# jeertmans/DiffeRT2d

Measured on AMD Instinct MI355X. Metric: ray-path candidates/s, higher is better.
Workload: dtype f32

## Files before the change

differt2d_amd/csrc/d2d.hip:

```cpp
#include <hip/hip_runtime.h>
#include <dlfcn.h>
#include <rccl/rccl.h>

#include <algorithm>
#include <cmath>
#include <cstdarg>
#include <cstdio>
#include <cstring>
#include <string>
#include <cstdlib>
#include <vector>

#include "../../include/d2d.h"
#define D2D_AUX_KERNELS 1
#include "d2d_launch.hpp"
#include "d2d_host.hpp"
#include "d2d_own.hpp"
#include "d2d_optgrad.hpp"
#include "d2d_optrev.hpp"

namespace d2d {

#define D2D_BY_MODE(fn, ...)                                   \
    switch (mode) {                                            \
// ... 273 lines not shown
        float tx = dx - ox, ty = dy - oy;
        float vx = ty, vy = -tx;
        float len = sqrtf(vx * vx + vy * vy);
        if (len == 0.0f) len = 1.0f;
        float nx = vx / len, ny = vy / len;
        float sq = tx * tx + ty * ty;
        if (sq == 0.0f) sq = 1.0f;
        refl[2 * j] = make_float4(ox, oy, nx, ny);
        refl[2 * j + 1] = make_float4(tx, ty, sq, len);
        const double rsq = 1.0 / (double)sq;
        flt[j] = make_float4((float)rsq, (float)(64.0 * 1.1920929e-07 * rsq), 0.0f, 0.0f);
    }
    int rc = c->d_refl.ensure(refl.size());
    if (rc) return rc;
    if ((rc = c->d_flt.ensure(flt.size()))) return rc;
    HIP_TRY(hipMemcpyAsync(c->d_flt.p, flt.data(), flt.size() * sizeof(float4), hipMemcpyHostToDevice, c->stream));
    if ((rc = c->d_kind.ensure((size_t)c->N + 1))) return rc;
    if ((rc = c->d_sincos.ensure((size_t)c->N + 1))) return rc;
    if ((rc = c->d_xys.ensure((size_t)c->N + 1))) return rc;
    if (c->N > 0) HIP_TRY(hipMemcpyAsync(c->d_xys.p, c->xys.data(), (size_t)c->N * sizeof(float4), hipMemcpyHostToDevice, c->stream));
    std::vector<float2> sc((size_t)c->N + 1);
    for (int j = 0; j < c->N; ++j) sc[(size_t)j] = make_float2(sinf(c->phi[j]), cosf(c->phi[j]));
    HIP_TRY(hipMemcpyAsync(c->d_refl.p, refl.data(), refl.size() * sizeof(float4), hipMemcpyHostToDevice, c->stream));
    if (c->N > 0) {
        HIP_TRY(hipMemcpyAsync(c->d_kind.p, c->kind.data(), (size_t)c->N, hipMemcpyHostToDevice, c->stream));
        HIP_TRY(hipMemcpyAsync(c->d_sincos.p, sc.data(), (size_t)c->N * sizeof(float2), hipMemcpyHostToDevice, c->stream));
    }
    HIP_TRY(hipStreamSynchronize(c->stream));
    return D2D_OK;
}

int upload_occl(d2d_ctx* c, float patch) {
    if (c->occl_patch == patch && c->d_occl.p) return D2D_OK;
    std::vector<float4> occl((size_t)c->N + 1);
    for (int j = 0; j < c->N; ++j) {
        const float* w = &c->xys[4 * (size_t)j];
        float ox = w[0], oy = w[1], dx = w[2], dy = w[3];
        float tx = dx - ox, ty = dy - oy;
        float ptx = patch * tx, pty = patch * ty;
        float p1x = ox - ptx, p1y = oy - pty;
        float p2x = dx + ptx, p2y = dy + pty;
        occl[j] = make_float4(p1x, p1y, p2x - p1x, p2y - p1y);
    }
    int rc = c->d_occl.ensure(occl.size());
    if (rc) return rc;
    HIP_TRY(hipMemcpyAsync(c->d_occl.p, occl.data(), occl.size() * sizeof(float4), hipMemcpyHostToDevice, c->stream));
    HIP_TRY(hipStreamSynchronize(c->stream));
    c->occl_patch = patch;
    return D2D_OK;
}

int upload_mask(d2d_ctx* c) {
    c->cw.clear();
    for (int j = 0; j < c->N; ++j)
        if (c->allowed[j]) c->cw.push_back(j);
    int rc = c->d_cw.ensure(c->cw.size() + 1);
    if (rc) return rc;
    if (!c->cw.empty()) {
        HIP_TRY(hipMemcpyAsync(c->d_cw.p, c->cw.data(), c->cw.size() * sizeof(int), hipMemcpyHostToDevice, c->stream));
        HIP_TRY(hipStreamSynchronize(c->stream));
    }
    return D2D_OK;
}

d2d::ObjTables obj_tables(d2d_ctx* c) {
    d2d::ObjTables T;
    T.occl = c->d_occl.p;
// ... 801 lines not shown
        if (c->stream) HIP_TRY(hipStreamSynchronize(c->stream));
        if (c->aux_stream) HIP_TRY(hipStreamSynchronize(c->aux_stream));
        if (c->sort_stream) HIP_TRY(hipStreamSynchronize(c->sort_stream));
        c->for_each_set([](d2d_ctx::PrepSet& sp) { sp.swept_pending = false; });
        c->last_small = small;
    }
    s.piped = c->pipeline && c->aux_stream != nullptr && s.d_stats == nullptr && !small;
    if (s.piped) {
        std::swap(c->cur, c->spare_sets[0]);
        for (int i = 0; i + 1 < d2d_ctx::N_SPARE; ++i) std::swap(c->spare_sets[i], c->spare_sets[i + 1]);
        s.set_was_swept = c->cur.swept_pending;
        if (c->cur.swept_pending) HIP_TRY(hipStreamWaitEvent(c->aux_stream, c->cur.ev_swept, 0));
        c->cur.swept_pending = false;
    }
    s.ps = s.piped ? c->aux_stream : c->stream;
    return D2D_OK;
}

static int sweep_args(d2d_ctx* c, Sweep& s) {
    const d2d_params* p = s.p;
    d2d::SweepArgs& a = s.a;
    memset(&a, 0, sizeof a);
    a.occl = c->d_occl.p;
    a.refl = c->d_refl.p;
    a.flt = c->d_flt.p;
    a.cw = c->d_cw.p;
    a.N = c->N;
    a.Nc = (int)c->cw.size();
    a.X = c->d_X.p;
    a.Y = c->d_Y.p;
    a.out = c->d_out.p;
    a.m = c->m;
    a.n = c->n;
    a.txx = s.tx[0];
    a.txy = s.tx[1];
    a.min_order = p->min_order;
    a.max_order = p->max_order;
    a.alpha = p->alpha;
    a.tol = p->tol;
    a.seg_lo = -p->seg_tol;
    a.seg_hi = 1.0f + p->seg_tol;
    const bool per_object = p->fun_id == D2D_FUN_RECEIVED_POWER_PER_OBJECT;
    s.th = d2d_host::sweep_thresholds(*p, s.grad_mode != 0, per_object ? c->coef.data() : nullptr, c->allowed.data(), c->N);
    a.coef = per_object ? c->d_coef.p : nullptr;
    a.flt_lo = s.th.flt_lo;
    a.flt_hi = s.th.flt_hi;
    a.on_lo = s.th.on_lo;
    a.on_hi = s.th.on_hi;
    a.loss_skip = s.th.loss_skip;
    for (int k = 0; k <= D2D_MAX_ORDER; ++k) a.fnum[k] = s.th.fnum[k];
    a.h2 = s.th.h2;
    a.sig_l2f = s.th.sig_l2f;
    a.sig_mono = s.th.sig_mono;
    a.fun_id = p->fun_id;
    a.cust_f = c->d_cust_f.p;
    a.cust_pb = c->d_cust_pb.p;
    a.cust_cells = (long)c->m * c->n;
    a.out_mode = p->out_mode;
    a.patch = p->patch;
    a.stats = s.d_stats;
    a.wave_cycles = (s.d_stats && c->want_wave_cycles) ? s.d_stats + D2D_NUM_STATS : nullptr;
    if (s.tiles > 0x7fffffffLL) return fail(D2D_ERR_INVALID, "grid too large: %lld tiles", s.tiles);
    s.grid_patches = dim3((unsigned)s.tiles);
    s.txg = p->grid_role == D2D_GRID_TX;
    const bool txg_cullable = s.txg && !c->txg_exhaustive && !(s.grad_mode && p->strict_nan);
    s.txg_culled = txg_cullable && s.th.degenerate_invalid;
// ... 127 lines not shown
    const size_t lds_l = (size_t)(3 * c->N + 1) * sizeof(float4) + 512;
    const size_t lds_r = (size_t)(3 * c->N + 1) * sizeof(float4) + (size_t)d2d::RL_GATHER * sizeof(unsigned long long);
    if (!rp.on || lds_l > d2d_host::LDS_LIMIT || lds_r > d2d_host::LDS_LIMIT) return D2D_OK;
    if (cur.d_rl_pool.ensure((size_t)rp.max_chunks * d2d::RL_CHUNK) != D2D_OK || cur.d_rl_next.ensure((size_t)rp.max_chunks) != D2D_OK) {
        (void)hipGetLastError();
        cur.d_rl_pool.release();
        cur.d_rl_next.release();
        c->rl_pool_mb = std::max<long long>(1, c->rl_pool_mb / 4);
        return D2D_OK;
    }
    const int orders = p->max_order - rp.k_lo + 1;
    const size_t per_order = (size_t)rp.leaf.slots + (size_t)rp.top.slots;
    if ((rc = cur.d_rl_idx.ensure(per_order * (size_t)orders))) return rc;
    int* const meta = reinterpret_cast<int*>(cur.d_shadow.p + c->N + d2d::SCHED_KEYS);
    cur.rl_meta_ptr = meta;
    if ((rc = cur.d_rl_meta.ensure((size_t)s.tiles))) return rc;
    if ((rc = cur.d_rl.ensure(1))) return rc;
    {
        const long long key[4] = {c->grid_version, rp.leaf.R, rp.top.R, (long long)c->m * 0x100000000ll + c->n};
        const size_t nbox = (size_t)rp.leaf.regions + (size_t)rp.top.regions;
        if (std::memcmp(key, c->rl_box_key, sizeof key) != 0 || c->d_rl_box.n < nbox) {
            if ((rc = c->d_rl_box.ensure(nbox))) return rc;
            hipLaunchKernelGGL(d2d::region_box_kernel, dim3((unsigned)rp.leaf.regions), dim3(256), 0, s.ps, c->d_X.p, c->d_Y.p,
                               c->m, c->n, rp.leaf.R, rp.leaf.regions_x, c->d_rl_box.p);
            hipLaunchKernelGGL(d2d::region_box_kernel, dim3((unsigned)rp.top.regions), dim3(256), 0, s.ps, c->d_X.p, c->d_Y.p,
                               c->m, c->n, rp.top.R, rp.top.regions_x, c->d_rl_box.p + rp.leaf.regions);
            HIP_TRY(hipGetLastError());
            std::memcpy(c->rl_box_key, key, sizeof key);
        }
    }
    auto fill = [](d2d::RegionLevel& l, const d2d_host::RegionLevelPlan& lp_) {
        l.S = lp_.S;
        l.R = lp_.R;
        l.regions_x = lp_.regions_x;
        l.regions_y = lp_.regions_y;
    };
    d2d::RegionLists rl;
    d2d::RegionLevel top;
    memset(&rl, 0, sizeof rl);
    memset(&top, 0, sizeof top);
    fill(rl.leaf, rp.leaf);
    fill(top, rp.top);
    rl.leaf.box = c->d_rl_box.p;
    top.box = c->d_rl_box.p + rp.leaf.regions;
    if ((rc = prep_hidden_masks(c, s, pr, rp, rl.leaf))) return rc;
    int* at = cur.d_rl_idx.p;
    int chunk_at = 0;
    for (int k = rp.k_lo; k <= p->max_order; ++k) {
        rl.leaf.cnt[k] = at; at += rp.leaf.slots;
        rl.leaf.chunk0[k] = chunk_at; chunk_at += (int)rp.leaf.slots;
        top.cnt[k] = at; at += rp.top.slots;
        top.chunk0[k] = chunk_at; chunk_at += (int)rp.top.slots;
    }
    rl.lp.pool = cur.d_rl_pool.p;
    rl.lp.next = cur.d_rl_next.p;
    rl.lp.head = meta + 1;
    rl.lp.n_static = (int)rp.n_static;
    rl.lp.max_chunks = (int)rp.max_chunks;
    rl.flag = meta + 2;
    a.fb_n = meta;
    a.fb_list = cur.d_rl_meta.p;
    if (!cur.rl_host_valid || std::memcmp(&rl, &cur.rl_host, sizeof rl) != 0) {
        cur.rl_host = rl;
        cur.rl_host_valid = true;
        hipLaunchKernelGGL(d2d::write_region_lists_kernel, dim3(1), dim3(1), 0, s.ps, cur.d_rl.p, rl);
        HIP_TRY(hipGetLastError());
// ... 1312 lines not shown
```

differt2d_amd/csrc/d2d_kernels.hpp:

```cpp
#pragma once
#include <hip/hip_runtime.h>
#include <stdint.h>

#include "../../include/d2d.h"

namespace d2d {

template <typename T>
__device__ __forceinline__ const __attribute__((address_space(4))) T* cmem(const T* p) {
    return (const __attribute__((address_space(4))) T*)(unsigned long long)p;
}

__device__ __forceinline__ float4 ldc4(const float4* p, long i) {
    typedef float v4f __attribute__((ext_vector_type(4)));
    const v4f v = ((const __attribute__((address_space(4))) v4f*)(unsigned long long)p)[i];
    return make_float4(v.x, v.y, v.z, v.w);
}
__device__ __forceinline__ int4 ldc4i(const int4* p, long i) {
    typedef int v4i __attribute__((ext_vector_type(4)));
    const v4i v = ((const __attribute__((address_space(4))) v4i*)(unsigned long long)p)[i];
    return make_int4(v.x, v.y, v.z, v.w);
}

template <typename T, unsigned OFF>
__device__ __forceinline__ T late_kernarg() {
    static_assert(sizeof(T) == 4 || sizeof(T) == 8, "one or two dwords");
    const auto base = __builtin_amdgcn_kernarg_segment_ptr();
    T v;
    if constexpr (sizeof(T) == 8) asm volatile("s_load_dwordx2 %0, %1, %2\n\ts_waitcnt lgkmcnt(0)" : "=s"(v) : "s"(base), "i"(OFF));
    else asm volatile("s_load_dword %0, %1, %2\n\ts_waitcnt lgkmcnt(0)" : "=s"(v) : "s"(base), "i"(OFF));
    return v;
}
#define D2D_LATE_ARG(T, field) late_kernarg<T, (unsigned)__builtin_offsetof(SweepArgs, field)>()

enum Mode { MODE_HARD = 0, MODE_HSIG = 1, MODE_SIG = 2 };

constexpr int RL_CHUNK = 128;
struct ListPool {
    unsigned long long* pool;
    int* next;
    int* head;
    int n_static;
    int max_chunks;
};
struct RegionLevel {
    int* cnt[D2D_MAX_ORDER + 1];
    int chunk0[D2D_MAX_ORDER + 1];
    int S;
    int R;
    int regions_x, regions_y;
    const float4* box;
    const unsigned long long* hidden;
    float hidden_dperp;
};
struct RegionLists {
    RegionLevel leaf;
    ListPool lp;
    int* flag;
};

struct SweepArgs {
    const RegionLists* __restrict__ rl;
    int* fb_n;
    int* fb_list;
    const float4* __restrict__ occl;
    const float4* __restrict__ refl;
    const float4* __restrict__ flt;
    const int* __restrict__ cw;
    int N, Nc;
    const float* __restrict__ X;
    const float* __restrict__ Y;
    float* __restrict__ out;
    int m, n;
    float txx, txy;
    int min_order, max_order;
    float alpha, tol;
    float seg_lo, seg_hi;
    float flt_lo, flt_hi;
    float on_lo, on_hi;
    float loss_skip;
    float sig_l2f;
    int sig_mono;
    const unsigned long long* __restrict__ shadow;
    float shadow_dperp;
    float shadow_lo, shadow_inv;
    int shadow_prefix_ok;
    const unsigned long long* __restrict__ pair;
    float pair_dperp;
    int pair_prefix_ok;
    float fnum[D2D_MAX_ORDER + 1];
    float h2;
    int fun_id;
    int out_mode;
    float patch;
    float* __restrict__ grad;
    const float* __restrict__ cot;
    float* __restrict__ partial;
    const float* __restrict__ cust_f;
    const float* __restrict__ cust_pb;
    long cust_cells;
    const float* __restrict__ coef;
    float* __restrict__ coef_partial;
    int coef_lds_off;

    const int* __restrict__ sched;
    int cullq_off;
// ... 403 lines not shown
        }
        if (K >= 2 && a.pair != nullptr) {
#pragma unroll
            for (int i = 0; i + 1 < K; ++i) {
                const unsigned long long m = HOIST ? pm_pre[i] : cmem(a.pair)[(size_t)cand[i] * a.N + cand[i + 1]];
                if (m != 0ull) {
                    const float k8 = 0.125f * a.shadow_inv;
                    const float ea_ = (sv[i] - padv[i] - a.shadow_lo) * k8, eb_ = (sv[i] + padv[i] - a.shadow_lo) * k8;
                    const float la_ = (sv[i + 1] - padv[i + 1] - a.shadow_lo) * k8, lb_ = (sv[i + 1] + padv[i + 1] - a.shadow_lo) * k8;
                    const bool ok = ea_ >= 0.0f && eb_ < 8.0f && la_ >= 0.0f && lb_ < 8.0f && 512.0f * eps * Ei[i] <= a.pair_dperp &&
                                    512.0f * eps * Ei[i + 1] <= a.pair_dperp;
                    const int ea = ok ? (int)ea_ : 0, eb = ok ? (int)eb_ : 0, la = ok ? (int)la_ : 0, lb = ok ? (int)lb_ : 0;
                    const bool all4 = ((m >> (ea + 8 * la)) & 1ull) && ((m >> (eb + 8 * la)) & 1ull) && ((m >> (ea + 8 * lb)) & 1ull) &&
                                      ((m >> (eb + 8 * lb)) & 1ull);
                    occl = occl || (ok && all4 && (eb - ea <= 1) && (lb - la <= 1));
                }
            }
        }
        if (wave_any(occl)) {
            if (MODE == MODE_HARD) hit_b = hit_b || occl;
            else if (MODE == MODE_HSIG) hit_c = occl ? 6.0f : hit_c;
            else {
                hit_z = occl ? 1.0e30f : hit_z;
                any_test = true;
            }
            active = active && (!occl || bad);
            D2D_WORK(2);
            if (!wave_any(active)) return;
        }
    }
    if (STATS) stat_add<2>(st, 1);
    constexpr bool PAIRS = MODE != MODE_SIG;
    if constexpr (PAIRS) {
    auto filt = [&](const float4& ww, int jj) -> unsigned {
        unsigned wbits = 0u;
#pragma unroll
        for (int i = 0; i <= K; ++i) {
            const int ig0 = (i == 0) ? -1 : cand[i - 1];
            const int ig1 = (i == K) ? -1 : cand[i];
            const bool skip = (jj == ig0 || jj == ig1);
            float Cx = ww.x - px[i], Cy = ww.y - py[i];
            float fa = by[i] * Cx - bx[i] * Cy;
            float fb = ww.z * Cy - ww.w * Cx;
            float fd = ww.w * bx[i] - ww.z * by[i];
            float pa = __builtin_fmaf(-a.flt_lo, fd, fa) * __builtin_fmaf(-a.flt_hi, fd, fa);
            float pb = __builtin_fmaf(-a.flt_lo, fd, fb) * __builtin_fmaf(-a.flt_hi, fd, fb);
            bool miss = fmaxf(pa, pb) > 0.0f;
            if (MODE == MODE_SIG && !skip) any_test = true;
            if (STATS) stat_add<4>(st, skip ? 0 : 1);
            wbits |= (!skip && active && (!miss || bad)) ? (1u << i) : 0u;
        }
        return wbits;
    };
    auto exact = [&](const float4& ww, int jj, unsigned wbits) {
#pragma unroll
        for (int i = 0; i <= K; ++i) {
            if (!wave_any((wbits >> i) & 1u)) continue;
            if (STATS) stat_add<5>(st, 1);
            D2D_WORK(2);
            const float Cx = ww.x - px[i], Cy = ww.y - py[i];
            const float fa = by[i] * Cx - bx[i] * Cy;
            const float fb = ww.z * Cy - ww.w * Cx;
            const float fd = ww.w * bx[i] - ww.z * by[i];
            bool dz = (fd == 0.0f);
            float dd = dz ? 1.0f : fd;
            float ta, tb;
            div2_exact(fa, fb, dd, ta, tb);
            ta = dz ? __builtin_inff() : ta;
            tb = dz ? __builtin_inff() : tb;
            if (MODE == MODE_HARD) {
                bool h = (ta >= a.seg_lo) && (ta <= a.seg_hi) && (tb >= a.seg_lo) && (tb <= a.seg_hi);
                hit_b = hit_b || h;
            } else if (MODE == MODE_HSIG) {
                nanflag = nanflag || (ta != ta) || (tb != tb);
                float c = fminf(fminf(clampact(ta - a.seg_lo, a.alpha), clampact(a.seg_hi - ta, a.alpha)),
                                fminf(clampact(tb - a.seg_lo, a.alpha), clampact(a.seg_hi - tb, a.alpha)));
                if (GRAD && (c > hit_c || (c == hit_c && hit_j >= 0 && (jj < hit_j || (jj == hit_j && i < hit_i))))) {
                    hit_i = i;
                    hit_j = jj;
                }
                if (GRAD) hit2 = (c > hit_c) ? hit_c : fmaxf(hit2, c);
                hit_c = fmaxf(hit_c, c);
            } else {
                nanflag = nanflag || (ta != ta) || (tb != tb);
                float z = fminf(fminf(a.alpha * (ta - a.seg_lo), a.alpha * (a.seg_hi - ta)),
                                fminf(a.alpha * (tb - a.seg_lo), a.alpha * (a.seg_hi - tb)));
                if (GRAD && (z > hit_z || (z == hit_z && hit_j >= 0 && (jj < hit_j || (jj == hit_j && i < hit_i))))) {
                    hit_i = i;
                    hit_j = jj;
                }
                if (GRAD) hit2 = (z > hit_z) ? hit_z : fmaxf(hit2, z);
                hit_z = fmaxf(hit_z, z);
            }
        }
        if (MODE == MODE_HARD) active = active && (!hit_b || bad);
        else if (MODE == MODE_HSIG) active = active && (hit_c != 6.0f || bad);
        else active = active && (hit_z < 17.5f || bad);
    };
    {
        bool done = a.N <= 0;
        if (!done && sh >= 0) {
            const unsigned b0 = filt(w, sh);
            D2D_WORK(K + 1);
            if (wave_any(b0 != 0u)) {
                exact(w, sh, b0);
                if (!wave_any(active)) {
                    st.shadow = sh;
                    done = true;
                }
            }
        }
        auto next_idx = [&](int x) -> int {
            ++x;
            return x == sh ? x + 1 : x;
        };
        int jA = (sh == 0) ? 1 : 0;
        if (!done && jA < a.N) {
            int jB = next_idx(jA);
            float4 wA = (sh >= 0) ? ldc4(a.occl, jA) : w;
            float4 wB = ldc4(a.occl, jB < a.N ? jB : jA);
            while (true) {
                const bool hasB = jB < a.N;
                const int nA = next_idx(jB), nB = next_idx(nA);
                const float4 wnA = ldc4(a.occl, nA < a.N ? nA : jA), wnB = ldc4(a.occl, nB < a.N ? nB : jA);
                const unsigned ba = filt(wA, jA);
                const unsigned bb = hasB ? filt(wB, jB) : 0u;
                D2D_WORK(hasB ? 2 * (K + 1) : (K + 1));
                if (wave_any((ba | bb) != 0u)) {
                    if (wave_any(ba != 0u)) {
                        exact(wA, jA, ba);
                        if (!wave_any(active)) {
                            st.shadow = jA;
                            break;
                        }
                    }
                    if (wave_any(bb != 0u)) {
                        exact(wB, jB, bb);
                        if (!wave_any(active)) {
                            st.shadow = jB;
                            break;
                        }
                    }
                }
                if (!(nA < a.N)) break;
                jA = nA;
                jB = nB;
                wA = wnA;
                wB = wnB;
            }
        }
    }
    } else {
    int nxt = sh >= 0 ? 0 : 1;
    if (nxt == sh) ++nxt;
    for (bool more = a.N > 0; more;) {
        const bool has_next = nxt < a.N;
        const float4 wn = ldc4(a.occl, has_next ? nxt : j);
        float fa_[K + 1], fb_[K + 1], fd_[K + 1];
        unsigned wbits = 0u;
#pragma unroll
        for (int i = 0; i <= K; ++i) {
            const int ig0 = (i == 0) ? -1 : cand[i - 1];
            const int ig1 = (i == K) ? -1 : cand[i];
            const bool skip = (j == ig0 || j == ig1);
            float Cx = w.x - px[i], Cy = w.y - py[i];
            float fa = by[i] * Cx - bx[i] * Cy;
            float fb = w.z * Cy - w.w * Cx;
            float fd = w.w * bx[i] - w.z * by[i];
            float pa = __builtin_fmaf(-a.flt_lo, fd, fa) * __builtin_fmaf(-a.flt_hi, fd, fa);
            float pb = __builtin_fmaf(-a.flt_lo, fd, fb) * __builtin_fmaf(-a.flt_hi, fd, fb);
            bool miss = fmaxf(pa, pb) > 0.0f;
            if (MODE == MODE_SIG && !skip) any_test = true;
            if (STATS) stat_add<4>(st, skip ? 0 : 1);
            wbits |= (!skip && active && (!miss || bad)) ? (1u << i) : 0u;
            fa_[i] = fa;
            fb_[i] = fb;
            fd_[i] = fd;
        }
        D2D_WORK(K + 1);
        if (wave_any(wbits != 0u)) {
#pragma unroll
            for (int i = 0; i <= K; ++i) {
// ... 1123 lines not shown
            int ce[D2D_MAX_ORDER] = {-1, -1, -1, -1};
            float ex[D2D_MAX_ORDER], ey[D2D_MAX_ORDER];
#pragma unroll
            for (int d = 0; d < K; ++d) {
                ce[d] = (int)((cu >> (12 * d)) & 0xfffull);
                ex[d] = __int_as_float(__builtin_amdgcn_readlane(__float_as_int(Ix[d]), b));
                ey[d] = __int_as_float(__builtin_amdgcn_readlane(__float_as_int(Iy[d]), b));
            }
            if (LIST) {
                float t = 0.0f;
                eval_candidate<K, MODE, STATS, GRAD, false, false>(a, ce, ex, ey, a.txx, a.txy, rxx, rxy, lane_bad, t, st, g);
                if (!(t == 0.0f)) sink->push(t);
            } else {
                eval_candidate<K, MODE, STATS, GRAD, false, false>(a, ce, ex, ey, a.txx, a.txy, rxx, rxy, lane_bad, acc, st, g);
            }
        }
        if (STATS) stat_add<14>(st, __builtin_amdgcn_s_memtime() - te0);
    }
}

template <int K, int MODE, bool STATS, bool GRAD, bool LIST, bool LISTED>
__device__ __forceinline__ void sweep_order_any(const SweepArgs& a, const float4* tab, const float (&bx)[4], const float (&by)[4],
                                                float rxx, float rxy, bool lane_bad, float& acc, WaveStats& st, GradCtx* g,
                                                long region, int part, int parts, ListSink* sink) {
    if constexpr (K >= 2 && LISTED) {
        sweep_order_listed<K, MODE, STATS, GRAD, LIST>(a, tab, bx, by, rxx, rxy, lane_bad, acc, st, g, region, part, parts, sink);
    } else {
        int lo = 0, hi = 0x7fffffff;
        if (parts > 1) first_wall_range(a, part, parts, lo, hi);
        sweep_order_culled<K, MODE, STATS, GRAD, LIST>(a, tab, bx, by, rxx, rxy, lane_bad, acc, st, g, lo, hi, sink);
    }
}

__device__ __forceinline__ long region_of(const SweepArgs& a, int tcol, int trow) {
    const int R = cmem(a.rl)->leaf.R;
    return (long)(trow / R) * cmem(a.rl)->leaf.regions_x + (tcol / R);
}

#if defined(__gfx942__) || defined(__gfx950__)
#define D2D_FENCE_FREE_HANDOVER 1
#else
#define D2D_FENCE_FREE_HANDOVER 0
#endif
constexpr int NAN_W = 16;
constexpr int NAN_R = 4;
constexpr int NAN_RY = NAN_W / NAN_R;
constexpr int NAN_LCAP = 2048;
constexpr int NAN_RB = NAN_LCAP / 64;
constexpr int NAN_WQCAP = 2048;
constexpr int HEAVY_PARTS = 4;
constexpr int TILE_W = 8;
constexpr int TILE_H = 8;

template <int MODE, bool STATS, int MAXK, bool GRADK, bool LISTED, bool SPARE = false>
__device__ __forceinline__ void fwd_patch(const SweepArgs& a, float4* tab, float* wl, const long b0_in, const bool from_queue) {
    const int lane = threadIdx.x & 63;
    const int tiles_x = (a.n + TILE_W - 1) / TILE_W;
    const bool scene = GRADK && a.partial != nullptr;
    float tbx_sum = 0.0f, tby_sum = 0.0f;
    WaveStats st;
#pragma unroll
    for (int i = 0; i < 16; ++i) st.c[i] = 0;
    st.shadow = -1;
    st.work = 0;
    const long n_items = (long)tiles_x * ((a.m + TILE_H - 1) / TILE_H) + (long)(HEAVY_PARTS - 1) * a.n_heavy;
    const bool exists = !SPARE || b0_in < n_items;
    const long b0 = exists ? b0_in : 0;
    const bool quarter = !STATS && !GRADK && MAXK == 2 && !from_queue && (b0 < (long)HEAVY_PARTS * a.n_heavy);
    const long tile0 = quarter ? (b0 / HEAVY_PARTS) : (b0 - (long)(HEAVY_PARTS - 1) * a.n_heavy);
    const int part = quarter ? (int)(b0 % HEAVY_PARTS) : 0;
    const long tile = from_queue ? b0 : (a.sched ? (long)a.sched[tile0] : tile0);
#ifdef D2D_AB_TIMELINE
    const unsigned long long t_line0 = __builtin_amdgcn_s_memrealtime();
    if (a.tl_ring && lane == 0 && !from_queue && b0_in == 0) a.tl_ring[2 * (a.tl_seq & 255)] = t_line0;
#endif
    const unsigned long long t_start = STATS ? __builtin_amdgcn_s_memtime() : 0ull;
    const int tcol = (int)(tile % tiles_x), trow = (int)(tile / tiles_x);
    const long region = LISTED ? region_of(a, tcol, trow) : 0;
    const int col = tcol * TILE_W + (lane & (TILE_W - 1));
    const int row = trow * TILE_H + (lane / TILE_W);
    const bool in_range = (col < a.n) && (row < a.m);
    const int ccol = col < a.n ? col : a.n - 1;
    const int crow = row < a.m ? row : a.m - 1;
    const long idx = (long)crow * a.n + ccol;
    const float rxx = a.X[idx], rxy = a.Y[idx];
    float* const cb = scene ? coef_acc_ptr(tab) : nullptr;
    if (scene) {
        for (int i = lane; i < 4 * a.N; i += 64) wl[i] = 0.0f;
        coef_acc_zero(cb, a.N);
        __syncthreads();
    }
    if (!exists) return;
    const bool lane_bad = !(fabsf(rxx) < 1e18f) || !(fabsf(rxy) < 1e18f) || !(fabsf(a.txx) < 1e18f) ||
                          !(fabsf(a.txy) < 1e18f);
    if (LISTED) {
        if (cmem(cmem(a.rl)->flag)[region] != 0 || wave_any(lane_bad)) {
            if (part == 0 && lane == 0) a.fb_list[atomicAdd(a.fb_n, 1)] = (int)tile;
            return;
        }
    }
    float acc = 0.0f;
    GradCtx g;
    g.grx = g.gry = g.tbx = g.tby = 0.0f;
    g.cot = in_range ? (a.cot ? a.cot[idx] : 1.0f) : 0.0f;
    g.wl = wl;
    g.cb = cb;
    g.scene = scene;
    g.ci = 0;
    g.cell = 0;
    float x0 = rxx, x1 = rxx, y0 = rxy, y1 = rxy;
#pragma unroll
    for (int off = 32; off > 0; off >>= 1) {
        x0 = fminf(x0, __shfl_xor(x0, off, 64));
        x1 = fmaxf(x1, __shfl_xor(x1, off, 64));
        y0 = fminf(y0, __shfl_xor(y0, off, 64));
        y1 = fmaxf(y1, __shfl_xor(y1, off, 64));
    }
    const bool box_ok = !wave_any(lane_bad);
    const float qn = __builtin_nanf("");
    const float bx[4] = {box_ok ? x0 : qn, x1, x1, x0};
    const float by[4] = {y0, y0, y1, y1};
    unsigned long long tq0 = STATS ? __builtin_amdgcn_s_memtime() : 0ull;
    if (STATS) stat_add<10>(st, tq0 - t_start);
#ifdef D2D_AB_TIMELINE
    const unsigned t_lineB = (unsigned)(__builtin_amdgcn_s_memrealtime() & 0xffffull);
    unsigned t_lineC = t_lineB;
#endif
    if (quarter) {
        const long hq = tile0 * HEAVY_PARTS + part;
        ListSink sink;
        sink.col = a.heavy_list + hq * (long)a.heavy_cap * 64 + lane;
        sink.cnt = 0;
        sink.over = false;
        sink.cap = a.heavy_cap;
        sink.through = true;
        float dummy = 0.0f;
        if (part == 0) {
            if (a.min_order <= 0 && a.max_order >= 0) {
                float t = 0.0f;
                sweep_order<0, MODE, false, false>(a, a.txx, a.txy, rxx, rxy, lane_bad, t, st, nullptr);
                if (!(t == 0.0f)) sink.push(t);
            }
            if (a.min_order <= 1 && a.max_order >= 1) {
                const unsigned long long* hid = LISTED ? cmem(a.rl)->leaf.hidden : nullptr;
                sweep_order_culled<1, MODE, false, false, true>(a, tab, bx, by, rxx, rxy, lane_bad, dummy, st, nullptr, 0, 0x7fffffff, &sink, nullptr,
                                                                hid ? hid + (size_t)region * a.N : nullptr, hid ? cmem(a.rl)->leaf.hidden_dperp : 0.0f);
            }
        }
#ifdef D2D_AB_TIMELINE
        t_lineC = (unsigned)(__builtin_amdgcn_s_memrealtime() & 0xffffull);
#endif
        if (a.min_order <= 2 && a.max_order >= 2)
            sweep_order_any<2, MODE, false, false, true, LISTED>(a, tab, bx, by, rxx, rxy, lane_bad, dummy, st, nullptr, region, part, HEAVY_PARTS, &sink);
        int* const heavy_cnt = D2D_LATE_ARG(int*, heavy_cnt);
        int* const heavy_done = D2D_LATE_ARG(int*, heavy_done);
        const int n_heavy_l = D2D_LATE_ARG(int, n_heavy), heavy_cap_l = D2D_LATE_ARG(int, heavy_cap);
        __hip_atomic_store(&heavy_cnt[hq * 64 + lane], sink.over ? -1 : sink.cnt, __ATOMIC_RELAXED, __HIP_MEMORY_SCOPE_AGENT);
        if (lane == 0) __hip_atomic_store(&heavy_cnt[(long)n_heavy_l * HEAVY_PARTS * 64 + hq], (int)st.work, __ATOMIC_RELAXED, __HIP_MEMORY_SCOPE_AGENT);
        int old = 0;
#if D2D_FENCE_FREE_HANDOVER
        __builtin_amdgcn_fence(__ATOMIC_RELEASE, "workgroup");
        __builtin_amdgcn_s_waitcnt(0x0F70);
        if (lane == 0) old = __hip_atomic_fetch_add(&heavy_done[tile0], 1, __ATOMIC_RELAXED, __HIP_MEMORY_SCOPE_AGENT);
#else
        if (lane == 0) old = __hip_atomic_fetch_add(&heavy_done[tile0], 1, __ATOMIC_RELEASE, __HIP_MEMORY_SCOPE_AGENT);
#endif
#ifdef D2D_AB_TIMELINE
        if (a.grad && lane == 0) {
            reinterpret_cast<unsigned*>(a.grad)[2 * b0] = (unsigned)(((t_line0 & 0xffffull) << 16) | (__builtin_amdgcn_s_memrealtime() & 0xffffull));
            reinterpret_cast<unsigned*>(a.grad)[2 * b0 + 1] = (t_lineB << 16) | t_lineC;
        }
#endif
        old = __builtin_amdgcn_readfirstlane(old);
        if (old != HEAVY_PARTS - 1) return;
#if !D2D_FENCE_FREE_HANDOVER
        __builtin_amdgcn_fence(__ATOMIC_ACQUIRE, "agent");
#endif
        unsigned work = 0;
        for (int q = 0; q < HEAVY_PARTS; ++q) {
            const long hq2 = tile0 * HEAVY_PARTS + q;
            int n = __hip_atomic_load(&heavy_cnt[hq2 * 64 + lane], __ATOMIC_RELAXED, __HIP_MEMORY_SCOPE_AGENT);
            const bool bad = n < 0 || n > heavy_cap_l;
            n = bad ? 0 : n;
            int nmax = n;
#pragma unroll
            for (int off = 32; off > 0; off >>= 1) nmax = max(nmax, __shfl_xor(nmax, off, 64));
            const int* col = reinterpret_cast<const int*>(D2D_LATE_ARG(float*, heavy_list)) + hq2 * (long)heavy_cap_l * 64 + lane;
            for (int i0 = 0; i0 < nmax; i0 += 8) {
                int v[8];
#pragma unroll
                for (int k = 0; k < 8; ++k)
                    v[k] = __hip_atomic_load(&col[(i0 + k < n ? i0 + k : 0) * 64], __ATOMIC_RELAXED, __HIP_MEMORY_SCOPE_AGENT);
#pragma unroll
                for (int k = 0; k < 8; ++k) acc = acc + (i0 + k < n ? __int_as_float(v[k]) : 0.0f);
            }
            if (bad) acc = __builtin_nanf("");
            work += (unsigned)__hip_atomic_load(&heavy_cnt[(long)n_heavy_l * HEAVY_PARTS * 64 + hq2], __ATOMIC_RELAXED, __HIP_MEMORY_SCOPE_AGENT);
        }
        st.work = work;
        if (lane == 0) __hip_atomic_store(&heavy_done[tile0], 0, __ATOMIC_RELAXED, __HIP_MEMORY_SCOPE_AGENT);
    } else {
    if (a.min_order <= 0 && a.max_order >= 0) sweep_order<0, MODE, STATS, GRADK>(a, a.txx, a.txy, rxx, rxy, lane_bad, acc, st, &g);
    unsigned long long tq1 = STATS ? __builtin_amdgcn_s_memtime() : 0ull;
    if (STATS) stat_add<11>(st, tq1 - tq0);
    if (a.min_order <= 1 && a.max_order >= 1) {
        const unsigned long long* hid = LISTED ? cmem(a.rl)->leaf.hidden : nullptr;
        sweep_order_culled<1, MODE, STATS, GRADK>(a, tab, bx, by, rxx, rxy, lane_bad, acc, st, &g, 0, 0x7fffffff, nullptr, nullptr,
                                                  hid ? hid + (size_t)region * a.N : nullptr, hid ? cmem(a.rl)->leaf.hidden_dperp : 0.0f);
    }
    unsigned long long tq2 = STATS ? __builtin_amdgcn_s_memtime() : 0ull;
    if (STATS) stat_add<12>(st, tq2 - tq1);
#ifdef D2D_AB_TIMELINE
    t_lineC = (unsigned)(__builtin_amdgcn_s_memrealtime() & 0xffffull);
// ... 10 lines not shown
            if (out_mode == D2D_OUT_ADD) {
                out[idx] = out[idx] + acc;
                if (GRADK) {
                    a.grad[2 * idx] = a.grad[2 * idx] + g.grx;
                    a.grad[2 * idx + 1] = a.grad[2 * idx + 1] + g.gry;
                }
            } else {
                out[idx] = acc;
                if (GRADK) {
                    a.grad[2 * idx] = g.grx;
                    a.grad[2 * idx + 1] = g.gry;
                }
            }
        }
    }
    if (scene) {
        tbx_sum += wave_sum(g.tbx);
        tby_sum += wave_sum(g.tby);
    }
    if (STATS && lane == 0 && a.wave_cycles) a.wave_cycles[tile] = __builtin_amdgcn_s_memtime() - t_start;
    if (!STATS) {
        unsigned* const cost_out = D2D_LATE_ARG(unsigned*, cost_out);
        if (cost_out && lane == 0) cost_out[tile] = st.work;
    }
#ifdef D2D_AB_TIMELINE
    if (!STATS && !GRADK && a.grad && lane == 0)
    if (!quarter) {
        reinterpret_cast<unsigned*>(a.grad)[2 * b0] = (unsigned)(((t_line0 & 0xffffull) << 16) | (__builtin_amdgcn_s_memrealtime() & 0xffffull));
        reinterpret_cast<unsigned*>(a.grad)[2 * b0 + 1] = (t_lineB << 16) | t_lineC;
    }
#endif
    if (scene) {
        __syncthreads();
        float* dst = a.partial + tile * (4 * a.N + 2);
        for (int i = lane; i < 4 * a.N; i += 64) dst[i] = wl[i];
        if (lane == 0) {
            dst[4 * a.N] = tbx_sum;
            dst[4 * a.N + 1] = tby_sum;
        }
        coef_acc_store(cb, a.N, tile);
    }
    if (STATS && a.stats) {
#pragma unroll
        for (int i = 0; i < 16; ++i) {
            unsigned v = st.c[i];
#pragma unroll
            for (int off = 32; off > 0; off >>= 1) v = max(v, (unsigned)__shfl_xor((int)v, off, 64));
            if (lane == 0) atomicAdd(&a.stats[i], (unsigned long long)v);
        }
    }
}

template <int MODE, bool STATS, int MAXK, bool GRADK = false, bool LISTED = false, int WPB = 1>
__global__ void __launch_bounds__(64 * WPB) power_fwd_kernel(SweepArgs a) {
    const int lane = threadIdx.x & 63;
    extern __shared__ float4 tab[];
    float* wl = reinterpret_cast<float*>(tab + 3 * a.N);
    if (!LISTED && a.fb_n != nullptr) {
        const int n = *a.fb_n;
        if (n > 0) {
            for (int i = lane; i < 2 * a.N; i += 64) tab[i] = ldc4(a.refl, i);
            for (int i = lane; i < a.N; i += 64) tab[2 * a.N + i] = ldc4(a.flt, i);
            __syncthreads();
        }
        for (int i = blockIdx.x; i < n; i += gridDim.x) {
            fwd_patch<MODE, STATS, MAXK, GRADK, false>(a, tab, wl, (long)a.fb_list[i], true);
            __syncthreads();
        }
        return;
    }
    for (int i = threadIdx.x; i < 2 * a.N; i += 64 * WPB) tab[i] = ldc4(a.refl, i);
    for (int i = threadIdx.x; i < a.N; i += 64 * WPB) tab[2 * a.N + i] = ldc4(a.flt, i);
    __syncthreads();
    fwd_patch<MODE, STATS, MAXK, GRADK, LISTED, (WPB > 1)>(a, tab, wl, WPB == 1 ? (long)blockIdx.x : (long)blockIdx.x * WPB + (threadIdx.x >> 6), false);
}

template <int K, int MODE, bool STATS, int W, bool LISTED>
__device__ __forceinline__ void split_order(const SweepArgs& a, const float4* tab, float* lists, int* meta,
                                            const float (&bx)[4], const float (&by)[4], float rxx, float rxy,
                                            bool lane_bad, float& acc, WaveStats& st, long region) {
    const int lane = threadIdx.x & 63, wv = threadIdx.x >> 6;
    int* cnts = meta;
    int* flags = meta + (W - 1) * 64;
    if (wv != 0) {
        ListSink sink;
        sink.col = lists + (size_t)(wv - 1) * SPLIT_LIST * 64 + lane;
        sink.cnt = 0;
        sink.over = false;
        float dummy = 0.0f;
        sweep_order_any<K, MODE, STATS, false, true, LISTED>(a, tab, bx, by, rxx, rxy, lane_bad, dummy, st, nullptr, region, wv, W, &sink);
        cnts[(wv - 1) * 64 + lane] = sink.cnt;
        const bool over = wave_any(sink.over);
        if (lane == 0) flags[wv - 1] = over ? 1 : 0;
    }
#pragma unroll 1
    for (int w = 0; w < W; ++w) {
        if (w == 1) __syncthreads();
        if (wv == 0) {
            if (w == 0 || flags[w - 1]) {
                sweep_order_any<K, MODE, STATS, false, false, LISTED>(a, tab, bx, by, rxx, rxy, lane_bad, acc, st, nullptr, region, w, W, nullptr);
            } else {
                const int n = cnts[(w - 1) * 64 + lane];
                int nmax = n;
#pragma unroll
                for (int off = 32; off > 0; off >>= 1) nmax = max(nmax, __shfl_xor(nmax, off, 64));
                const float* col = lists + (size_t)(w - 1) * SPLIT_LIST * 64 + lane;
                for (int i = 0; i < nmax; ++i)
// ... 613 lines not shown
    if (a.min_order <= 1 && a.max_order >= 1) {
        const unsigned long long* hid = LISTED ? cmem(a.rl)->leaf.hidden : nullptr;
        sweep_order_culled_txg<1, MODE, GRADK>(a, tab, bx, by, cx, cy, lane_bad, acc, st, &g, 0, 0x7fffffff, nullptr,
                                               hid ? hid + (size_t)region * a.N : nullptr, hid ? cmem(a.rl)->leaf.hidden_dperp : 0.0f);
    }
    if constexpr (LISTED) {
        if (a.min_order <= 2 && a.max_order >= 2) sweep_order_listed_txg<2, MODE, GRADK>(a, tab, bx, by, cx, cy, lane_bad, acc, st, &g, region);
        if (MAXK >= 3 && a.min_order <= 3 && a.max_order >= 3) sweep_order_listed_txg<3, MODE, GRADK>(a, tab, bx, by, cx, cy, lane_bad, acc, st, &g, region);
        if (MAXK >= 4 && a.min_order <= 4 && a.max_order >= 4) sweep_order_listed_txg<4, MODE, GRADK>(a, tab, bx, by, cx, cy, lane_bad, acc, st, &g, region);
    } else {
        if (a.min_order <= 2 && a.max_order >= 2) sweep_order_culled_txg<2, MODE, GRADK>(a, tab, bx, by, cx, cy, lane_bad, acc, st, &g);
        if (MAXK >= 3 && a.min_order <= 3 && a.max_order >= 3) sweep_order_culled_txg<3, MODE, GRADK>(a, tab, bx, by, cx, cy, lane_bad, acc, st, &g);
        if (MAXK >= 4 && a.min_order <= 4 && a.max_order >= 4) sweep_order_culled_txg<4, MODE, GRADK>(a, tab, bx, by, cx, cy, lane_bad, acc, st, &g);
    }
    if (in_range) {
        if (a.out_mode == D2D_OUT_ADD) {
            a.out[idx] = a.out[idx] + acc;
            if (GRADK) {
                a.grad[2 * idx] = a.grad[2 * idx] + g.grx;
                a.grad[2 * idx + 1] = a.grad[2 * idx + 1] + g.gry;
            }
        } else {
            a.out[idx] = acc;
            if (GRADK) {
                a.grad[2 * idx] = g.grx;
                a.grad[2 * idx + 1] = g.gry;
            }
        }
    }
    if (a.cost_out && lane == 0) a.cost_out[tile] = st.work;
    if (scene) {
        const float sx = wave_sum(g.tbx), sy = wave_sum(g.tby);
        __syncthreads();
        float* dst = a.partial + tile * (4 * a.N + 2);
        for (int i = lane; i < 4 * a.N; i += 64) dst[i] = wl[i];
        if (lane == 0) {
            dst[4 * a.N] = sx;
            dst[4 * a.N + 1] = sy;
        }
        coef_acc_store(cb, a.N, tile);
    }
}

template <int MODE, int MAXK, bool GRADK = false, bool LISTED = false>
__global__ void __launch_bounds__(64) power_fwd_txg_kernel(SweepArgs a) {
    const int lane = threadIdx.x & 63;
    extern __shared__ float4 tab[];
    float* wl = reinterpret_cast<float*>(tab + 3 * a.N);
    if (!LISTED && a.fb_n != nullptr) {
        const int n = *a.fb_n;
        if (n > 0) {
            for (int i = lane; i < 2 * a.N; i += 64) tab[i] = ldc4(a.refl, i);
            for (int i = lane; i < a.N; i += 64) tab[2 * a.N + i] = ldc4(a.flt, i);
            __syncthreads();
        }
        for (int i = blockIdx.x; i < n; i += gridDim.x) {
            txg_patch<MODE, MAXK, GRADK, false>(a, tab, wl, (long)a.fb_list[i], true);
            __syncthreads();
        }
        return;
    }
    for (int i = lane; i < 2 * a.N; i += 64) tab[i] = ldc4(a.refl, i);
    for (int i = lane; i < a.N; i += 64) tab[2 * a.N + i] = ldc4(a.flt, i);
    __syncthreads();
    txg_patch<MODE, MAXK, GRADK, LISTED>(a, tab, wl, (long)blockIdx.x, false);
}

// ... 1287 lines not shown
```

Baseline: 28480 billion.

## Restructure occluder scan with paired loads, lazy own-wall masking, fast division

In the non-gradient occlusion path, the loop now reads occluders two at a time with one 32-byte scalar load. It no longer skips the shadowing wall index through next_idx, and it drops the per-test own-wall comparison, masking own-candidate bits only when the scan reaches a candidate's wall pair. The occluder buffer is padded and zero-filled so the lookahead load stays in bounds. Tile and region index math switches from 64-bit division to precomputed 32-bit multiply-shift division, with readfirstlane to keep the indices scalar. The risk is that the shadowing wall is now rescanned, and the reciprocal-based division is only exact within certain ranges.

```diff
diff --git a/differt2d_amd/csrc/d2d.hip b/differt2d_amd/csrc/d2d.hip
--- a/differt2d_amd/csrc/d2d.hip
+++ b/differt2d_amd/csrc/d2d.hip
@@ -329,7 +329,7 @@
 
 int upload_occl(d2d_ctx* c, float patch) {
     if (c->occl_patch == patch && c->d_occl.p) return D2D_OK;
-    std::vector<float4> occl((size_t)c->N + 1);
+    std::vector<float4> occl((((size_t)c->N + 1) & ~(size_t)1) + 2, make_float4(0.0f, 0.0f, 0.0f, 0.0f));
     for (int j = 0; j < c->N; ++j) {
         const float* w = &c->xys[4 * (size_t)j];
         float ox = w[0], oy = w[1], dx = w[2], dy = w[3];
@@ -1197,6 +1197,7 @@
     a.out = c->d_out.p;
     a.m = c->m;
     a.n = c->n;
+    a.tiles_x_div = d2d::make_div((uint32_t)s.tiles_x);
     a.txx = s.tx[0];
     a.txy = s.tx[1];
     a.min_order = p->min_order;
@@ -1390,6 +1391,7 @@
     auto fill = [](d2d::RegionLevel& l, const d2d_host::RegionLevelPlan& lp_) {
         l.S = lp_.S;
         l.R = lp_.R;
+        l.R_div = d2d::make_div((uint32_t)lp_.R);
         l.regions_x = lp_.regions_x;
         l.regions_y = lp_.regions_y;
     };
diff --git a/differt2d_amd/csrc/d2d_div.hpp b/differt2d_amd/csrc/d2d_div.hpp
--- /dev/null
+++ b/differt2d_amd/csrc/d2d_div.hpp
@@ -0,0 +1,42 @@
+#pragma once
+#include <stdint.h>
+
+namespace d2d {
+
+struct DivU32 {
+    uint32_t d;
+    uint32_t mul;
+    uint32_t shift;
+};
+
+constexpr DivU32 make_div(uint32_t d) {
+    DivU32 v = {d ? d : 1u, 0u, 0u};
+    if ((v.d & (v.d - 1u)) == 0u) {
+        while ((1u << v.shift) != v.d) ++v.shift;
+    } else {
+        v.mul = (uint32_t)((1ull << 32) / v.d);
+    }
+    return v;
+}
+
+__attribute__((always_inline)) constexpr void divmod(const DivU32& v, uint32_t n, uint32_t& q, uint32_t& r) {
+    if (v.mul == 0u) {
+        q = n >> v.shift;
+        r = n & (v.d - 1u);
+    } else {
+        q = (uint32_t)(((uint64_t)n * v.mul) >> 32);
+        r = n - q * v.d;
+        if (r >= v.d) {
+            ++q;
+            r -= v.d;
+        }
+    }
+}
+
+__attribute__((always_inline)) constexpr uint32_t div_by(const DivU32& v, uint32_t n) {
+    uint32_t q = 0, r = 0;
+    divmod(v, n, q, r);
+    return q;
+}
+
+}
diff --git a/differt2d_amd/csrc/d2d_kernels.hpp b/differt2d_amd/csrc/d2d_kernels.hpp
--- a/differt2d_amd/csrc/d2d_kernels.hpp
+++ b/differt2d_amd/csrc/d2d_kernels.hpp
@@ -3,6 +3,7 @@
 #include <stdint.h>
 
 #include "../../include/d2d.h"
+#include "d2d_div.hpp"
 
 namespace d2d {
 
@@ -16,6 +17,14 @@
     const v4f v = ((const __attribute__((address_space(4))) v4f*)(unsigned long long)p)[i];
     return make_float4(v.x, v.y, v.z, v.w);
 }
+__device__ __forceinline__ void ldc4x2(const float4* p, unsigned byte_off, float4& r0, float4& r1) {
+    typedef float v8f __attribute__((ext_vector_type(8)));
+    const v8f v = *(const __attribute__((address_space(4))) v8f*)((unsigned long long)p + byte_off);
+    r0 = make_float4(v.s0, v.s1, v.s2, v.s3);
+    r1 = make_float4(v.s4, v.s5, v.s6, v.s7);
+}
+struct FlagOn { static constexpr bool value = true; };
+struct FlagOff { static constexpr bool value = false; };
 __device__ __forceinline__ int4 ldc4i(const int4* p, long i) {
     typedef int v4i __attribute__((ext_vector_type(4)));
     const v4i v = ((const __attribute__((address_space(4))) v4i*)(unsigned long long)p)[i];
@@ -49,6 +58,7 @@
     int S;
     int R;
     int regions_x, regions_y;
+    DivU32 R_div;
     const float4* box;
     const unsigned long long* hidden;
     float hidden_dperp;
@@ -72,6 +82,7 @@
     const float* __restrict__ Y;
     float* __restrict__ out;
     int m, n;
+    DivU32 tiles_x_div;
     float txx, txy;
     int min_order, max_order;
     float alpha, tol;
@@ -541,13 +552,14 @@
     if (STATS) stat_add<2>(st, 1);
     constexpr bool PAIRS = MODE != MODE_SIG;
     if constexpr (PAIRS) {
-    auto filt = [&](const float4& ww, int jj) -> unsigned {
+    auto filt = [&](const float4& ww, int jj, auto own_c) -> unsigned {
+        constexpr bool OWN = decltype(own_c)::value;
         unsigned wbits = 0u;
 #pragma unroll
         for (int i = 0; i <= K; ++i) {
             const int ig0 = (i == 0) ? -1 : cand[i - 1];
             const int ig1 = (i == K) ? -1 : cand[i];
-            const bool skip = (jj == ig0 || jj == ig1);
+            const bool skip = OWN && (jj == ig0 || jj == ig1);
             float Cx = ww.x - px[i], Cy = ww.y - py[i];
             float fa = by[i] * Cx - bx[i] * Cy;
             float fb = ww.z * Cy - ww.w * Cx;
@@ -609,7 +621,7 @@
     {
         bool done = a.N <= 0;
         if (!done && sh >= 0) {
-            const unsigned b0 = filt(w, sh);
+            const unsigned b0 = filt(w, sh, FlagOn());
             D2D_WORK(K + 1);
             if (wave_any(b0 != 0u)) {
                 exact(w, sh, b0);
@@ -619,6 +631,62 @@
                 }
             }
         }
+        if constexpr (!GRAD) {
+        if (!done) {
+            int own_nxt = 0x7fffffff;
+#pragma unroll
+            for (int d = 0; d < K; ++d) own_nxt = min(own_nxt, cand[d] & ~1);
+            int jA = 0;
+            float4 wA, wB;
+            ldc4x2(a.occl, 0u, wA, wB);
+            while (true) {
+                float4 wnA, wnB;
+                ldc4x2(a.occl, (unsigned)(jA + 2) << 4, wnA, wnB);
+                const int jB = jA + 1;
+                const bool hasB = jB < a.N;
+                unsigned ba = filt(wA, jA, FlagOff());
+                unsigned bb = hasB ? filt(wB, jB, FlagOff()) : 0u;
+                D2D_WORK(hasB ? 2 * (K + 1) : (K + 1));
+                unsigned own_tests = 0u;
+                if (K > 0 && jA == own_nxt) {
+                    unsigned ma = 0u, mb = 0u;
+                    int nxt = 0x7fffffff;
+#pragma unroll
+                    for (int d = 0; d < K; ++d) {
+                        ma |= (cand[d] == jA) ? (3u << d) : 0u;
+                        mb |= (cand[d] == jB) ? (3u << d) : 0u;
+                        const int o = cand[d] & ~1;
+                        nxt = min(nxt, o > jA ? o : 0x7fffffff);
+                    }
+                    own_nxt = nxt;
+                    ba &= ~ma;
+                    bb &= ~mb;
+                    own_tests = (unsigned)(__builtin_popcount(ma) + (hasB ? __builtin_popcount(mb) : 0));
+                }
+                if (STATS) stat_add<4>(st, 0ull - own_tests);
+                if (wave_any((ba | bb) != 0u)) {
+                    if (wave_any(ba != 0u)) {
+                        exact(wA, jA, ba);
+                        if (!wave_any(active)) {
+                            st.shadow = jA;
+                            break;
+                        }
+                    }
+                    if (wave_any(bb != 0u)) {
+                        exact(wB, jB, bb);
+                        if (!wave_any(active)) {
+                            st.shadow = jB;
+                            break;
+                        }
+                    }
+                }
+                jA += 2;
+                if (!(jA < a.N)) break;
+                wA = wnA;
+                wB = wnB;
+            }
+        }
+        } else {
         auto next_idx = [&](int x) -> int {
             ++x;
             return x == sh ? x + 1 : x;
@@ -632,8 +700,8 @@
                 const bool hasB = jB < a.N;
                 const int nA = next_idx(jB), nB = next_idx(nA);
                 const float4 wnA = ldc4(a.occl, nA < a.N ? nA : jA), wnB = ldc4(a.occl, nB < a.N ? nB : jA);
-                const unsigned ba = filt(wA, jA);
-                const unsigned bb = hasB ? filt(wB, jB) : 0u;
+                const unsigned ba = filt(wA, jA, FlagOn());
+                const unsigned bb = hasB ? filt(wB, jB, FlagOn()) : 0u;
                 D2D_WORK(hasB ? 2 * (K + 1) : (K + 1));
                 if (wave_any((ba | bb) != 0u)) {
                     if (wave_any(ba != 0u)) {
@@ -657,6 +725,7 @@
                 wA = wnA;
                 wB = wnB;
             }
+        }
         }
     }
     } else {
@@ -1846,9 +1915,10 @@
     }
 }
 
-__device__ __forceinline__ long region_of(const SweepArgs& a, int tcol, int trow) {
-    const int R = cmem(a.rl)->leaf.R;
-    return (long)(trow / R) * cmem(a.rl)->leaf.regions_x + (tcol / R);
+__device__ __forceinline__ int region_of(const SweepArgs& a, int tcol, int trow) {
+    const auto* rd = &cmem(a.rl)->leaf.R_div;
+    const DivU32 R = {rd->d, rd->mul, rd->shift};
+    return (int)(div_by(R, (unsigned)trow) * (unsigned)cmem(a.rl)->leaf.regions_x + div_by(R, (unsigned)tcol));
 }
 
 #if defined(__gfx942__) || defined(__gfx950__)
@@ -1867,9 +1937,9 @@
 constexpr int TILE_H = 8;
 
 template <int MODE, bool STATS, int MAXK, bool GRADK, bool LISTED, bool SPARE = false>
-__device__ __forceinline__ void fwd_patch(const SweepArgs& a, float4* tab, float* wl, const long b0_in, const bool from_queue) {
+__device__ __forceinline__ void fwd_patch(const SweepArgs& a, float4* tab, float* wl, const unsigned b0_in, const bool from_queue) {
     const int lane = threadIdx.x & 63;
-    const int tiles_x = (a.n + TILE_W - 1) / TILE_W;
+    const DivU32 tiles_x = a.tiles_x_div;
     const bool scene = GRADK && a.partial != nullptr;
     float tbx_sum = 0.0f, tby_sum = 0.0f;
     WaveStats st;
@@ -1877,20 +1947,22 @@
     for (int i = 0; i < 16; ++i) st.c[i] = 0;
     st.shadow = -1;
     st.work = 0;
-    const long n_items = (long)tiles_x * ((a.m + TILE_H - 1) / TILE_H) + (long)(HEAVY_PARTS - 1) * a.n_heavy;
+    const unsigned n_items = tiles_x.d * ((unsigned)(a.m + TILE_H - 1) / TILE_H) + (unsigned)(HEAVY_PARTS - 1) * (unsigned)a.n_heavy;
     const bool exists = !SPARE || b0_in < n_items;
-    const long b0 = exists ? b0_in : 0;
-    const bool quarter = !STATS && !GRADK && MAXK == 2 && !from_queue && (b0 < (long)HEAVY_PARTS * a.n_heavy);
-    const long tile0 = quarter ? (b0 / HEAVY_PARTS) : (b0 - (long)(HEAVY_PARTS - 1) * a.n_heavy);
+    const unsigned b0 = exists ? (unsigned)__builtin_amdgcn_readfirstlane((int)b0_in) : 0u;
+    const bool quarter = !STATS && !GRADK && MAXK == 2 && !from_queue && (b0 < (unsigned)HEAVY_PARTS * (unsigned)a.n_heavy);
+    const int tile0 = (int)(quarter ? (b0 / HEAVY_PARTS) : (b0 - (unsigned)(HEAVY_PARTS - 1) * (unsigned)a.n_heavy));
     const int part = quarter ? (int)(b0 % HEAVY_PARTS) : 0;
-    const long tile = from_queue ? b0 : (a.sched ? (long)a.sched[tile0] : tile0);
+    const int tile = __builtin_amdgcn_readfirstlane(from_queue ? (int)b0 : (a.sched ? a.sched[tile0] : tile0));
 #ifdef D2D_AB_TIMELINE
     const unsigned long long t_line0 = __builtin_amdgcn_s_memrealtime();
     if (a.tl_ring && lane == 0 && !from_queue && b0_in == 0) a.tl_ring[2 * (a.tl_seq & 255)] = t_line0;
 #endif
     const unsigned long long t_start = STATS ? __builtin_amdgcn_s_memtime() : 0ull;
-    const int tcol = (int)(tile % tiles_x), trow = (int)(tile / tiles_x);
-    const long region = LISTED ? region_of(a, tcol, trow) : 0;
+    unsigned tcol_u, trow_u;
+    divmod(tiles_x, (unsigned)tile, trow_u, tcol_u);
+    const int tcol = (int)tcol_u, trow = (int)trow_u;
+    const int region = LISTED ? region_of(a, tcol, trow) : 0;
     const int col = tcol * TILE_W + (lane & (TILE_W - 1));
     const int row = trow * TILE_H + (lane / TILE_W);
     const bool in_range = (col < a.n) && (row < a.m);
@@ -1909,7 +1981,7 @@
                           !(fabsf(a.txy) < 1e18f);
     if (LISTED) {
         if (cmem(cmem(a.rl)->flag)[region] != 0 || wave_any(lane_bad)) {
-            if (part == 0 && lane == 0) a.fb_list[atomicAdd(a.fb_n, 1)] = (int)tile;
+            if (part == 0 && lane == 0) a.fb_list[atomicAdd(a.fb_n, 1)] = tile;
             return;
         }
     }
@@ -1941,9 +2013,9 @@
     unsigned t_lineC = t_lineB;
 #endif
     if (quarter) {
-        const long hq = tile0 * HEAVY_PARTS + part;
+        const int hq = tile0 * HEAVY_PARTS + part;
         ListSink sink;
-        sink.col = a.heavy_list + hq * (long)a.heavy_cap * 64 + lane;
+        sink.col = a.heavy_list + (long)hq * (long)a.heavy_cap * 64 + lane;
         sink.cnt = 0;
         sink.over = false;
         sink.cap = a.heavy_cap;
@@ -1969,7 +2041,7 @@
         int* const heavy_cnt = D2D_LATE_ARG(int*, heavy_cnt);
         int* const heavy_done = D2D_LATE_ARG(int*, heavy_done);
         const int n_heavy_l = D2D_LATE_ARG(int, n_heavy), heavy_cap_l = D2D_LATE_ARG(int, heavy_cap);
-        __hip_atomic_store(&heavy_cnt[hq * 64 + lane], sink.over ? -1 : sink.cnt, __ATOMIC_RELAXED, __HIP_MEMORY_SCOPE_AGENT);
+        __hip_atomic_store(&heavy_cnt[(long)hq * 64 + lane], sink.over ? -1 : sink.cnt, __ATOMIC_RELAXED, __HIP_MEMORY_SCOPE_AGENT);
         if (lane == 0) __hip_atomic_store(&heavy_cnt[(long)n_heavy_l * HEAVY_PARTS * 64 + hq], (int)st.work, __ATOMIC_RELAXED, __HIP_MEMORY_SCOPE_AGENT);
         int old = 0;
 #if D2D_FENCE_FREE_HANDOVER
@@ -1992,7 +2064,7 @@
 #endif
         unsigned work = 0;
         for (int q = 0; q < HEAVY_PARTS; ++q) {
-            const long hq2 = tile0 * HEAVY_PARTS + q;
+            const long hq2 = (long)tile0 * HEAVY_PARTS + q;
             int n = __hip_atomic_load(&heavy_cnt[hq2 * 64 + lane], __ATOMIC_RELAXED, __HIP_MEMORY_SCOPE_AGENT);
             const bool bad = n < 0 || n > heavy_cap_l;
             n = bad ? 0 : n;
@@ -2069,7 +2141,7 @@
 #endif
     if (scene) {
         __syncthreads();
-        float* dst = a.partial + tile * (4 * a.N + 2);
+        float* dst = a.partial + (long)tile * (4 * a.N + 2);
         for (int i = lane; i < 4 * a.N; i += 64) dst[i] = wl[i];
         if (lane == 0) {
             dst[4 * a.N] = tbx_sum;
@@ -2101,7 +2173,7 @@
             __syncthreads();
         }
         for (int i = blockIdx.x; i < n; i += gridDim.x) {
-            fwd_patch<MODE, STATS, MAXK, GRADK, false>(a, tab, wl, (long)a.fb_list[i], true);
+            fwd_patch<MODE, STATS, MAXK, GRADK, false>(a, tab, wl, (unsigned)a.fb_list[i], true);
             __syncthreads();
         }
         return;
@@ -2109,7 +2181,7 @@
     for (int i = threadIdx.x; i < 2 * a.N; i += 64 * WPB) tab[i] = ldc4(a.refl, i);
     for (int i = threadIdx.x; i < a.N; i += 64 * WPB) tab[2 * a.N + i] = ldc4(a.flt, i);
     __syncthreads();
-    fwd_patch<MODE, STATS, MAXK, GRADK, LISTED, (WPB > 1)>(a, tab, wl, WPB == 1 ? (long)blockIdx.x : (long)blockIdx.x * WPB + (threadIdx.x >> 6), false);
+    fwd_patch<MODE, STATS, MAXK, GRADK, LISTED, (WPB > 1)>(a, tab, wl, WPB == 1 ? blockIdx.x : blockIdx.x * WPB + (threadIdx.x >> 6), false);
 }
 
 template <int K, int MODE, bool STATS, int W, bool LISTED>
@@ -2789,7 +2861,7 @@
     if (scene) {
         const float sx = wave_sum(g.tbx), sy = wave_sum(g.tby);
         __syncthreads();
-        float* dst = a.partial + tile * (4 * a.N + 2);
+        float* dst = a.partial + (long)tile * (4 * a.N + 2);
         for (int i = lane; i < 4 * a.N; i += 64) dst[i] = wl[i];
         if (lane == 0) {
             dst[4 * a.N] = sx;
```

Measured after the change: 30460 billion (median of 6 runs). +7.0%, better.
